# erererq/gym-lorenz

Hardware: NVIDIA B200
Metric: env_steps_per_sec (higher is better)
Workload: dtype f64

## Files before the change

gym_lorenz_b200/csrc/chaos_b200.cu:

```cuda
#include <math.h>
#include <pthread.h>
#include <sched.h>
#include <stdarg.h>
#include <time.h>
#include <stdio.h>
#include <stdlib.h>
#include <string.h>

#include "kernels_common.cuh"
#include "host_copy.h"

cudaError_t cl_launch_derivatives(int kind, const void* state, const float* action, void* out,
                                  int64_t n, cudaStream_t st);

using cl::KParams;

struct CopyHelper;

namespace {

const cl_layout kLayouts[CL_ENV_KIND_COUNT] = {
     {8, 4, 0, 6, 3, 0, -500.0, 500.0, -HUGE_VAL, HUGE_VAL, 0, 0},
     {8, 10, 0, 6, 3, 0, -500.0, 500.0, -HUGE_VAL, HUGE_VAL, 0, 0},
     {8, 9, 0, 8, 3, 0, -2.0, 2.0, -HUGE_VAL, HUGE_VAL, 0, 0},
// ... 306 lines not shown
  if (r == CL_OK) ctx->step_index += 1;
  return r;
}

extern "C" int cl_step(cl_ctx* ctx, void* stream, const cl_buffers* buf, const cl_io* io) {
  if (!ctx) return fail(nullptr, CL_EINVAL, "null ctx");
  if (!io || !io->action) return fail(ctx, CL_EINVAL, "cl_step: io.action is required");
  KParams p;
  int r = fill_params(ctx, buf, io, p);
  if (r) return r;
  p.reward_f32 = 0;
  CU(cudaSetDevice(ctx->cfg.device));
  r = launch(ctx, p, cl::MODE_STEP, (cudaStream_t)stream);
  if (r == CL_OK) ctx->step_index += 1;
  return r;
}

typedef CUresult (*encode_tiled_fn)(CUtensorMap*, CUtensorMapDataType, cuuint32_t, void*, const cuuint64_t*,
                                    const cuuint64_t*, const cuuint32_t*, const cuuint32_t*, CUtensorMapInterleave,
                                    CUtensorMapSwizzle, CUtensorMapL2promotion, CUtensorMapFloatOOBfill);
static bool action_tensor_map(CUtensorMap* out, const float* base, uint64_t n_x, uint64_t n_ch, uint64_t T,
                              uint64_t row_stride, uint64_t t_stride, uint32_t chunk) {
  static encode_tiled_fn fn = nullptr;
  static bool tried = false;
  if (!tried) {
    tried = true;
    void* f = nullptr;
    cudaDriverEntryPointQueryResult q;
    if (cudaGetDriverEntryPoint("cuTensorMapEncodeTiled", &f, cudaEnableDefault, &q) == cudaSuccess &&
        q == cudaDriverEntryPointSuccess)
      fn = (encode_tiled_fn)f;
  }
  if (!fn || chunk < 1 || chunk > 256 || n_ch > 256 || T < chunk) return false;
  const cuuint64_t dims[3] = {n_x, n_ch, T};
  const cuuint64_t strides[2] = {row_stride * sizeof(float), t_stride * sizeof(float)};
  const cuuint32_t box[3] = {32, (cuuint32_t)n_ch, chunk};
  const cuuint32_t estr[3] = {1, 1, 1};
  return fn(out, CU_TENSOR_MAP_DATA_TYPE_FLOAT32, 3, (void*)base, dims, strides, box, estr, CU_TENSOR_MAP_INTERLEAVE_NONE,
            CU_TENSOR_MAP_SWIZZLE_NONE, CU_TENSOR_MAP_L2_PROMOTION_NONE, CU_TENSOR_MAP_FLOAT_OOB_FILL_NONE) == CUDA_SUCCESS;
}

static bool want_dynamic(const cl_ctx* ctx, int T, int chunk) {
  const char* ov = getenv("CHAOS_B200_DYN");
  if (ov && ov[0] == '0') return false;
  const int64_t W = (ctx->cfg.num_envs + 31) / 32, nsched = (int64_t)ctx->sm_count * 4;
  if (T < 2 * chunk) return false;
  if (ov && ov[0] == '1') return true;
  if (W <= nsched) return false;
  if (W * (int64_t)((T + chunk - 1) / chunk) >= (int64_t)1 << 31) return false;
  const double eff = (double)W / (double)(((W + nsched - 1) / nsched) * nsched);
  return eff < 0.95;
}

extern "C" int cl_rollout(cl_ctx* ctx, void* stream, const cl_buffers* buf, const cl_io* io,
                          const cl_rollout_desc* d) {
  if (!ctx) return fail(nullptr, CL_EINVAL, "null ctx");
  if (!io || !d || d->T < 1) return fail(ctx, CL_EINVAL, "cl_rollout: io/desc required, T >= 1");
  if (io->noise) return fail(ctx, CL_EINVAL, "cl_rollout: noise override is single-step only");
  KParams p;
  int r = fill_params(ctx, buf, io, p);
  if (r) return r;
  p.T = d->T; p.act_ts = d->act_ts; p.obs_ts = d->obs_ts; p.rew_ts = d->rew_ts; p.done_ts = d->done_ts;
  p.synth_amp = (float)d->synth_amp;
  cudaStream_t st = (cudaStream_t)stream;
  CU(cudaSetDevice(ctx->cfg.device));
  int chunk = CL_DYN_CHUNK_DEFAULT;
  if (const char* ov = getenv("CHAOS_B200_DYN_CHUNK")) { const int c = atoi(ov); if (c >= 1 && c <= 16) chunk = c; }
  int mode = cl::MODE_ROLLOUT;
  alignas(64) CUtensorMap tmap;
  if (want_dynamic(ctx, d->T, chunk)) {
    const int64_t W = (ctx->cfg.num_envs + 31) / 32;
    if (!ctx->dyn_bps) {
      int occ = 0;
      cudaError_t e = is_parity(ctx->cfg.kind) ? cl_dyn_occupancy_parity(ctx->cfg.kind, chunk, &occ)
                                               : cl_dyn_occupancy_northstar(ctx->cfg.kind, chunk, &occ);
      if (e != cudaSuccess) return fail(ctx, CL_ECUDA, "dyn occupancy query: %s", cudaGetErrorString(e));
      int bps = (int)(W / ((int64_t)ctx->sm_count * 4));
      bps = bps < 1 ? 1 : (bps > 4 ? 4 : bps);
      if (const char* ov = getenv("CHAOS_B200_DYN_BPS")) { const int b = atoi(ov); if (b >= 1 && b <= 16) bps = b; }
      ctx->dyn_bps = occ < bps ? occ : bps;
    }
    if (ctx->dyn_bps >= 1) {
      CU(cudaMemsetAsync(ctx->d_dyn, 0, sizeof(uint32_t) * (size_t)(W + 1), st));
      p.dyn_counter = ctx->d_dyn;
      p.dyn_progress = ctx->d_dyn + 1;
      p.dyn_chunk = chunk;
      p.dyn_nchunks = (d->T + chunk - 1) / chunk;
      p.dyn_nwarps = (int32_t)W;
      const int64_t workers = (int64_t)ctx->sm_count * ctx->dyn_bps;
      const int64_t tasks = W * (int64_t)((d->T + chunk - 1) / chunk);
      p.dyn_grid = (int32_t)(workers * 4 < tasks ? workers : (tasks + 3) / 4);
      p.dyn_tma = (io->action != nullptr && io->act_es == 1 && (io->act_cs % 4) == 0 && (d->act_ts % 4) == 0 &&
                   ((uintptr_t)io->action % 16) == 0 && io->act_cs >= W * 32) ? 1 : 0;
      {
        const char* ov = getenv("CHAOS_B200_SM");
        if (!(ov && ov[0] == '0') && p.dyn_tma) {
          const int grid = (int)(W < ctx->sm_count ? W : ctx->sm_count);
          const int qn = (int)(W / grid), cmax = (int)((W + grid - 1) / grid);
          int workers = qn >= 4 ? 4 * (qn / 4) : qn;
          workers = workers > 16 ? 16 : workers;
          if (workers == 16 && qn < 20) workers = 12;
          if (const char* w = getenv("CHAOS_B200_SM_WORKERS")) { const int k = atoi(w); if (k >= 1 && k <= 16) workers = k < qn ? k : qn; }
          int sc = 16;
          const size_t per_warp = (size_t)ctx->lay.n_state * 32u * (size_t)ctx->lay.real_bytes + 32u * 12u + 28u;
          while (sc > 1 && (size_t)cmax * (2u * (size_t)sc * (size_t)ctx->lay.act_dim * 128u + per_warp) + 256u > 200u * 1024u) sc /= 2;
          if (const char* w = getenv("CHAOS_B200_SM_CHUNK")) { const int k = atoi(w); if (k >= 1 && k <= 16) sc = k; }
          if (sc > d->T) sc = d->T;
          if (cmax <= 64) {
            p.sm_grid = grid; p.sm_workers = workers; p.sm_chunk = sc;
            p.sm_gdiv = 1;
            if (const char* w = getenv("CHAOS_B200_SM_GDIV")) { const int k = atoi(w); if (k >= 1 && k <= 16) p.sm_gdiv = k; }
            p.host_tmap = &tmap;
            p.sm_tmap_ok = action_tensor_map(&tmap, io->action, (uint64_t)W * 32, (uint64_t)ctx->lay.act_dim,
                                             (uint64_t)d->T, (uint64_t)io->act_cs, (uint64_t)d->act_ts, (uint32_t)sc) ? 1 : 0;
            const char* tm = getenv("CHAOS_B200_SM_TMAP");
            if (tm && tm[0] == '0') p.sm_tmap_ok = 0;
          }
        }
      }
      mode = cl::MODE_ROLLOUT_DYN;
      ctx->dyn_launches += 1;
    }
  }
  r = launch(ctx, p, mode, st);
  if (r == CL_OK) ctx->step_index += (uint64_t)d->T;
  return r;
}

static int check_policy_kind(cl_ctx* ctx, const char* fn, int kind) {
  if (kind == CL_ENV_HR_SYNC || kind == CL_ENV_PMSM_SYNC) return CL_OK;
  return fail(ctx, CL_EINVAL, "%s: env kind %d is not supported (hr_sync and pmsm_sync only)", fn, kind);
}

static int policy_prelude(cl_ctx* ctx, const char* fn, const char* objs, bool objs_ok, const cl_io* io,
                          const cl_rollout_desc* d, const cl_policy* pol, bool need_last) {
  if (!ctx) return fail(nullptr, CL_EINVAL, "null ctx");
  const int r = check_policy_kind(ctx, fn, ctx->cfg.kind);
  if (r) return r;
  if (ctx->cfg.flags & CL_F_OBS_F64) return fail(ctx, CL_EINVAL, "%s: float32 observations only", fn);
  if (!io || !d || !pol || !objs_ok || d->T < 1) return fail(ctx, CL_EINVAL, "%s: %s required, T >= 1", fn, objs);
  if (io->action || io->noise) return fail(ctx, CL_EINVAL, "%s: io.action and io.noise must be NULL", fn);
  if (!pol->params || !pol->obs0 || (need_last && !pol->obs_last))
    return fail(ctx, CL_EINVAL, need_last ? "%s: params, obs0 and obs_last are required"
                                          : "%s: params and obs0 are required", fn);
  return CL_OK;
}

static int policy_params(cl_ctx* ctx, const cl_buffers* buf, const cl_io* io, const cl_rollout_desc* d,
                         KParams& p) {
  const int r = fill_params(ctx, buf, io, p);
  if (r) return r;
  p.T = d->T; p.obs_ts = d->obs_ts; p.rew_ts = d->rew_ts; p.done_ts = d->done_ts;
  CU(cudaSetDevice(ctx->cfg.device));
  return CL_OK;
}

static bool collect_complete(const cl_collect* col) {
  return col->starts && col->obs && col->actions && col->rewards && col->values && col->log_probs &&
         col->episode_starts && col->last_values;
}

static int policy_done(cl_ctx* ctx, cudaStream_t st, cudaError_t e, const char* what, int T) {
  if (e != cudaSuccess) return fail(ctx, CL_ECUDA, "%s launch failed: %s", what, cudaGetErrorString(e));
  ctx->launches += 1;
// ... 497 lines not shown
```

gym_lorenz_b200/csrc/kernels_common.cuh:

```cuda
#pragma once
#include <cuda.h>
#include <cuda_runtime.h>
#include <stdint.h>
#include <string.h>

#include "../../include/chaos_b200.h"
#include "philox.cuh"

namespace cl {

struct KParams {
  int64_t n, n_pad, env_id_base;
  int64_t i_begin;
  uint32_t k0, k1;
  uint64_t step_index;
  uint64_t* step_ptr;
  int32_t max_steps, substeps, flags, reward_f32;
  double dt, alpha, act_limit, act_gain, param_jitter;
  void* state;
  int32_t* aux_int;
  int32_t* ep_len;
  double* ep_return;
  double* stats;
  const float* action;
  int64_t act_es, act_cs;
  const double* noise;
  void* obs;
  int64_t obs_es, obs_cs;
  void* reward;
  uint8_t* done;
  void* term_obs;
  double* last_ep_ret;
  int32_t* last_ep_len;
  const uint8_t* mask;
  uint8_t* warp_done;
  int32_t host_rows;
  const uint32_t* act_ready;
  uint32_t act_gen;
  int32_t act_slice_envs;
  int32_t act_lane_slices;
  const uint32_t* act_host_words;
  int32_t act_lanes, act_nslices;
  uint32_t* host_err;
  int32_t T;
  int64_t act_ts, obs_ts, rew_ts, done_ts;
  float synth_amp;
  const float* bc1;
  const float* bc2;
  int32_t bc1_n, bc2_n;
  double h, hh, h3, h6;
  float hf, hhf, h3f, h6f;
  double nom[3];
  float nomf[3];
  double nom_br;
  float nom_brf;
  float act_limit_f, act_gain_f;
  uint32_t* dyn_counter;
  uint32_t* dyn_progress;
  int32_t dyn_chunk, dyn_nchunks, dyn_nwarps, dyn_tma, dyn_grid;
  int32_t sm_grid, sm_workers, sm_chunk, sm_gdiv;
  int32_t sm_tmap_ok;
  const CUtensorMap* host_tmap;
  int32_t rows_fast;
  int32_t no_plain;
  int32_t* host_plain_out;
};

enum LaunchMode { MODE_STEP = 0, MODE_ROLLOUT = 1, MODE_RESET = 2, MODE_INIT = 3, MODE_ROLLOUT_DYN = 4 };


__device__ __forceinline__ float clipf(float a, float lo, float hi) {
  return a < lo ? lo : (a > hi ? hi : a);
}
__device__ __forceinline__ double clipd(double a, double lo, double hi) {
  return a < lo ? lo : (a > hi ? hi : a);
}

__device__ __forceinline__ double pow_pos(double x, double a) {
  if (a == 0.5) return sqrt(x);
  if (a == 1.0 / 3) return cbrt(x);
  if (!(a > 0.0) || !(a < 64.0)) return pow(x, a);
  if (x == 0.0) return 0.0;
  return exp(a * log(x));
}

__device__ __forceinline__ double mul_keep(double a, double b) { return __dmul_rn(a, b); }
__device__ __forceinline__ float mul_keep(float a, float b) { return a * b; }
__device__ __forceinline__ double mul_rn(double a, double b) { return __dmul_rn(a, b); }
__device__ __forceinline__ float mul_rn(float a, float b) { return __fmul_rn(a, b); }

__device__ __forceinline__ Stream make_stream(const KParams& p, int64_t i, uint64_t step) {
  const uint64_t gid = (uint64_t)(p.env_id_base + i);
  Stream s;
  s.id_lo = (uint32_t)gid;
  s.id_hi = (uint32_t)(gid >> 32);
  s.step = (uint32_t)step;
  s.k0 = p.k0;
  s.k1 = p.k1 ^ (uint32_t)((step >> 32) & 0x00FFFFFFu);
  return s;
}

__device__ __forceinline__ uint64_t step_base(const KParams& p) {
  return p.step_ptr != nullptr ? *((volatile const uint64_t*)p.step_ptr) : p.step_index;
}
__global__ void k_advance_step(uint64_t* step, uint64_t count);
__global__ void k_relay(const uint32_t* host_words, uint32_t* dev_words, uint32_t gen, uint32_t lanes, uint32_t spl,
                        uint32_t nslices, uint32_t* host_err);

template <int N>
__device__ __forceinline__ void draw_uniform(const Stream& rng, uint32_t tag, double lo, double hi,
                                             double* out) {
#pragma unroll
  for (int b = 0; b < (N + 1) / 2; ++b) {
    const u32x4 r = rng.draw(tag + (uint32_t)b);
    out[2 * b] = uniform53(r.x, r.y, lo, hi);
    if (2 * b + 1 < N) out[2 * b + 1] = uniform53(r.z, r.w, lo, hi);
  }
}
// ... 560 lines not shown
      phase ^= 1u;
    }
    const float* ab = abuf;
    unsigned bad_acc = 0u;
    bool fin = E::finite(s);
    PlainPending<E> pend;
    pend.begin(p, i, t0);
    auto intervals = [&](auto spec_tag) {
      constexpr int SPEC = decltype(spec_tag)::value;
      for (int tl = 0; tl < len; ++tl) {
        const int t = t0 + tl;
        const uint64_t step = step0 + (uint64_t)t;
        float a[E::ACT];
        if (!PLAIN && p.action == nullptr) {
          synth_action<E>(p, make_stream(p, i, step), a);
        } else if (tma) {
#pragma unroll
          for (int cc = 0; cc < E::ACT; ++cc) a[cc] = ab[(tl * E::ACT + cc) * 32 + lane];
        } else {
#pragma unroll
          for (int cc = 0; cc < E::ACT; ++cc)
            a[cc] = live ? p.action[(int64_t)t * p.act_ts + i * p.act_es + cc * p.act_cs] : 0.0f;
        }
        env_interval<E, true, PLAIN, SPEC, true>(s, ep_len, ep_ret, p, i, live, lane, t, step, a, want_noise, obs64, autoreset, bad_acc, sm_rows, fin, &pend);
      }
    };
    if constexpr (PLAIN) {
      if (E::spec(s, p) == 1) intervals(SpecTag<1>{});
      else intervals(SpecTag<0>{});
    } else {
      intervals(SpecTag<0>{});
    }
    if (bad_acc && lane == 0) atomicAdd(&p.stats[CL_STAT_NONFINITE], (double)bad_acc);
    bad_acc = 0u;
    if (live) {
      E::store(s, p, i);
      p.ep_len[i] = ep_len;
      p.ep_return[i] = ep_ret;
    }
    __syncwarp();
    if (lane == 0) st_release_u32(p.dyn_progress + e, c + 1u);
    if constexpr (PLAIN) {
      if (CL_PLAIN_DEFER) plain_emit<E, true>(p, i, live, pend);
    }
    q = grab();
  }
}



template <class E>
struct SmLayout {
  typedef typename E::real real;
  size_t act, state, ep_ret, ep_len, mbar, prog, total;
  __host__ __device__ SmLayout(int cnt, int chunk) {
    size_t o = 0;
    act = o;    o += (size_t)cnt * 2 * chunk * E::ACT * 32 * sizeof(float);
    state = o;  o += (size_t)cnt * E::NSTATE * 32 * sizeof(real);
    ep_ret = o; o += (size_t)cnt * 32 * sizeof(double);
    ep_len = o; o += (size_t)cnt * 32 * sizeof(int32_t);
    mbar = o;   o += (size_t)cnt * 3 * sizeof(uint64_t);
    prog = o;   o += ((size_t)cnt + 1) * sizeof(uint32_t);
    total = (o + 127) & ~(size_t)127;
  }
};

__device__ __forceinline__ void tma_load_3d(void* dst, const void* tmap, int x, int y, int z, uint64_t* bar) {
  asm volatile(
      "cp.async.bulk.tensor.3d.shared::cluster.global.tile.mbarrier::complete_tx::bytes [%0], [%1, {%2, %3, %4}], [%5];"
      ::"r"(smem_u32(dst)), "l"(tmap), "r"(x), "r"(y), "r"(z), "r"(smem_u32(bar))
      : "memory");
}

#ifndef CL_SM_THREADS
#define CL_SM_THREADS 576
#endif
#ifndef CL_SM_MINB
#define CL_SM_MINB 0
#endif
template <class E>
__global__ void __launch_bounds__(CL_SM_THREADS, CL_SM_MINB) k_rollout_sm(const KParams p,
                                                                         const __grid_constant__ CUtensorMap tmap) {
  typedef typename E::real real;
  extern __shared__ __align__(128) unsigned char sm_raw[];
  const unsigned lane = threadIdx.x & 31u;
  const int wib = threadIdx.x >> 5, nres = blockDim.x >> 5;
  const int W = p.dyn_nwarps, G = (int)gridDim.x, b = (int)blockIdx.x;
  const int qn = W / G, rn = W % G;
  const int e0 = b * qn + (b < rn ? b : rn);
  const int cnt = qn + (b < rn ? 1 : 0);
  const int cmax = qn + (rn ? 1 : 0);
  const int ng = cnt - nres;
  const int Tc = p.sm_chunk, Tg = max(1, Tc / max(1, p.sm_gdiv));
  const int nchunks = 1 + (p.T - 1 + Tc - 1) / Tc;
  const int nchunks_g = 1 + (p.T - 1 + Tg - 1) / Tg;
  auto chunk_t0 = [&](int f, int c, int tc) { return c == 0 ? 0 : min(p.T, f + (c - 1) * tc); };
  auto chunk_len = [&](int f, int c, int tc) { return min(c == 0 ? f : tc, p.T - chunk_t0(f, c, tc)); };
  const SmLayout<E> L(cmax, Tc);
  float* const act = (float*)(sm_raw + L.act);
  real* const st = (real*)(sm_raw + L.state);
  double* const s_ret = (double*)(sm_raw + L.ep_ret);
  int32_t* const s_len = (int32_t*)(sm_raw + L.ep_len);
  uint64_t* const mbar = (uint64_t*)(sm_raw + L.mbar);
  volatile uint32_t* const prog = (volatile uint32_t*)(sm_raw + L.prog);
  uint32_t* const counter = (uint32_t*)(sm_raw + L.prog) + cmax;
  const int per_buf = Tc * E::ACT * 32;

  for (int k = threadIdx.x; k < cnt * 3; k += blockDim.x) mbar_init(&mbar[k], 1);
  for (int k = threadIdx.x; k <= cmax; k += blockDim.x) ((uint32_t*)(sm_raw + L.prog))[k] = 0u;
  for (int k = threadIdx.x; k < cnt * 32; k += blockDim.x) {
    const int le = k >> 5, ln = k & 31;
    const int64_t i = (int64_t)(e0 + le) * 32 + ln;
#pragma unroll
    for (int c = 0; c < E::NSTATE; ++c) st[(le * E::NSTATE + c) * 32 + ln] = ldp<real>(p, c, i);
    s_ret[k] = __ldcg(p.ep_return + i);
    s_len[k] = __ldcg(p.ep_len + i);
  }
  asm volatile("fence.mbarrier_init.release.cluster;" ::: "memory");
  __syncthreads();

  auto stage = [&](int le, int f, int c, int tc) {
    const int t0 = chunk_t0(f, c, tc);
    uint64_t* bar = &mbar[le * 3 + (c & 1)];
    float* dst = act + (size_t)(le * 2 + (c & 1)) * per_buf;
    if (p.sm_tmap_ok) {
      if (lane == 0) {
        mbar_expect_tx(bar, (uint32_t)(per_buf * sizeof(float)));
        tma_load_3d(dst, &tmap, (e0 + le) * 32, 0, t0, bar);
      }
    } else {
      const int len = chunk_len(f, c, tc);
      if (lane == 0) mbar_expect_tx(bar, (uint32_t)(len * E::ACT * 128));
      __syncwarp();
      for (int k = (int)lane; k < len * E::ACT; k += 32) {
        const int tl = k / E::ACT, cc = k % E::ACT;
        const float* src = p.action + (int64_t)(t0 + tl) * p.act_ts + (int64_t)cc * p.act_cs + (int64_t)(e0 + le) * 32;
        bulk_g2s(dst + (tl * E::ACT + cc) * 32, src, 128u, bar);
      }
    }
  };
  auto wait_actions = [&](int le, int c) {
    uint64_t* bar = &mbar[le * 3 + (c & 1)];
    const uint32_t parity = (uint32_t)(c >> 1) & 1u;
    uint32_t spins = 0;
    while (!mbar_try_wait(bar, parity)) spin_guard(spins);
  };
  for (int le = wib; le < cnt; le += nres) { const int tc = le < nres ? Tc : Tg; stage(le, 1 + le * tc / cnt, 0, tc); }

  const uint64_t step0 = step_base(p);
  unsigned bad_acc = 0u;

  auto run_chunk = [&](typename E::S& s, int32_t& ep_len, double& ep_ret, bool& fin, PlainPending<E>& pend,
                       const int le, const int c, const int t0, const int len, const int64_t i, const bool live) {
    const float* ab = act + (size_t)(le * 2 + (c & 1)) * per_buf;
    auto intervals = [&](auto spec_tag) {
      constexpr int SPEC = decltype(spec_tag)::value;
      for (int tl = 0; tl < len; ++tl) {
        const int t = t0 + tl;
        const uint64_t step = step0 + (uint64_t)t;
        float a[E::ACT];
#pragma unroll
        for (int cc = 0; cc < E::ACT; ++cc) a[cc] = ab[(tl * E::ACT + cc) * 32 + lane];
        env_interval<E, true, true, SPEC, true>(s, ep_len, ep_ret, p, i, live, lane, t, step, a, false, false, true,
                                                bad_acc, nullptr, fin, &pend);
      }
    };
    if (E::spec(s, p) == 1) intervals(SpecTag<1>{});
    else intervals(SpecTag<0>{});
  };

  const uint32_t g_total = (uint32_t)ng * (uint32_t)nchunks_g;
  const int g_credit = ng * (Tc / Tg);
  typename E::S s = {};
  int32_t ep_len = 0;
  double ep_ret = 0.0;
  bool fin = true;
  PlainPending<E> pend;
  pend.valid = 0u;
  int in_regs = -1;
  int c_own = 0;
  int credit = (wib * g_credit) % nres;
  bool guests_left = ng > 0, want_guest = false;
  for (;;) {
    int le, c;
    bool guest;
    if (want_guest) {
      uint32_t q = 0;
      if (lane == 0) q = atomicAdd(counter, 1u);
      q = __shfl_sync(0xffffffffu, q, 0);
      if (q >= g_total) { guests_left = false; want_guest = false; continue; }
      guest = true; le = nres + (int)(q % (uint32_t)ng); c = (int)(q / (uint32_t)ng);
    } else if (c_own < nchunks) {
      guest = false; le = wib; c = c_own;
    } else if (guests_left) {
      want_guest = true;
      continue;
    } else {
      break;
    }
    const int tc = guest ? Tg : Tc, nch = guest ? nchunks_g : nchunks;
    const int f = 1 + le * tc / cnt;
    const int t0 = chunk_t0(f, c, tc), len = chunk_len(f, c, tc);
    const int64_t i = (int64_t)(e0 + le) * 32 + lane;
    const bool live = i < p.n;
    if (guest && c > 0) {
      uint32_t spins = 0;
      if (lane == 0) {
        while (prog[le] != (uint32_t)c) { __nanosleep(32); spin_guard(spins); }
      }
      __syncwarp();
      uint64_t* hb = &mbar[le * 3 + 2];
      const uint32_t parity = (uint32_t)(c - 1) & 1u;
      while (!mbar_try_wait(hb, parity)) spin_guard(spins);
    }
    if (c + 1 < nch) stage(le, f, c + 1, tc);
    if (in_regs != le) {
      E::load_sm(s, st + (size_t)le * E::NSTATE * 32, lane);
      ep_len = s_len[le * 32 + lane];
      ep_ret = s_ret[le * 32 + lane];
      E::prepare(s, p, live);
      fin = E::finite(s);
      pend.begin(p, i, t0);
      in_regs = le;
    }
    wait_actions(le, c);
    run_chunk(s, ep_len, ep_ret, fin, pend, le, c, t0, len, i, live);
    bool park;
    if (guest) {
      park = true;
      want_guest = false;
    } else {
      c_own += 1;
      credit += g_credit;
      want_guest = guests_left && credit >= nres && c_own < nchunks;
      if (want_guest) credit -= nres;
      park = want_guest || c_own == nchunks;
    }
    if (park) {
      E::store_sm(s, st + (size_t)le * E::NSTATE * 32, lane);
      s_len[le * 32 + lane] = ep_len;
      s_ret[le * 32 + lane] = ep_ret;
      if (guest) {
        __syncwarp();
        if (lane == 0) {
          prog[le] = (uint32_t)c + 1u;
          mbar_arrive(&mbar[le * 3 + 2]);
        }
      }
      if (CL_PLAIN_DEFER) plain_emit<E, true>(p, i, live, pend);
      pend.valid = 0u;
      in_regs = -1;
    }
  }
  if (bad_acc && lane == 0) atomicAdd(&p.stats[CL_STAT_NONFINITE], (double)bad_acc);

  __syncthreads();
  for (int k = threadIdx.x; k < cnt * 32; k += blockDim.x) {
    const int le = k >> 5, ln = k & 31;
    const int64_t i = (int64_t)(e0 + le) * 32 + ln;
    if (i < p.n) {
#pragma unroll
      for (int c = 0; c < E::NSTATE; ++c) stp<real>(p, c, i, st[(le * E::NSTATE + c) * 32 + ln]);
      p.ep_return[i] = s_ret[k];
      p.ep_len[i] = s_len[k];
    }
  }
}

template <class E>
__global__ void __launch_bounds__(256) k_reset(const KParams p) {
  typedef typename E::real real;
  const int64_t i = (int64_t)blockIdx.x * blockDim.x + threadIdx.x;
  const uint64_t step0 = step_base(p);
  if (i < p.n && (p.mask == nullptr || p.mask[i] != 0)) {
    typename E::S s = {};
    E::load(s, p, i);
    const Stream rng = make_stream(p, i, step0);
    real obs[E::OBS];
    E::reset(s, p, rng, obs);
    E::store(s, p, i);
    p.ep_len[i] = 0;
    p.ep_return[i] = 0.0;
    if (p.obs) store_obs<real>(p.obs, 0, p.obs_es, p.obs_cs, i, obs, E::OBS, (p.flags & CL_F_OBS_F64) != 0);
  }
}

template <class E>
__global__ void __launch_bounds__(256) k_init(const KParams p) {
  const int64_t i = (int64_t)blockIdx.x * blockDim.x + threadIdx.x;
  if (i >= p.n) return;
  typename E::S s = {};
  const Stream rng = make_stream(p, i, 0);
  E::init_persistent(s, p, rng);
  E::store(s, p, i);
  p.ep_len[i] = 0;
  p.ep_return[i] = 0.0;
}

template <class E>
inline bool rows_fast_ok(const KParams& p, bool rollout) {
  return p.obs != nullptr && !(p.flags & CL_F_OBS_F64) && p.obs_cs == 1 && p.obs_es == E::OBS &&
         ((uintptr_t)p.obs % 16) == 0 && (!rollout || (p.obs_ts % 4) == 0) &&
         ((uintptr_t)p.term_obs % 16) == 0;
}

template <class E>
inline bool plain_rollout_ok(const KParams& p, int mode) {
  return PlainRollout<E>::value && !p.no_plain && E::NOISE == 0 && p.action != nullptr && p.obs != nullptr && p.obs_es == 1 &&
         p.obs_cs == p.n_pad && p.obs_ts == (int64_t)E::OBS * p.n_pad && p.rew_ts == p.n_pad && p.done_ts == p.n_pad &&
         !(p.flags & CL_F_OBS_F64) && !p.rows_fast && p.reward != nullptr && !p.reward_f32 && p.done != nullptr &&
         p.term_obs == nullptr &&
         (p.flags & CL_F_AUTORESET) && (mode != MODE_ROLLOUT_DYN || p.dyn_tma);
}

template <class E>
cudaError_t launch_env(const KParams& p_in, int mode, cudaStream_t st, int block) {
  KParams p = p_in;
  const bool roll = (mode == MODE_ROLLOUT || mode == MODE_ROLLOUT_DYN);
  p.rows_fast = (mode == MODE_STEP || roll) && rows_fast_ok<E>(p, roll) ? 1 : 0;
  constexpr bool HAS_PLAIN = PlainRollout<E>::value != 0;
  const bool plain = roll && plain_rollout_ok<E>(p, mode);
  if (p.host_plain_out) *p.host_plain_out = plain ? 1 : 0;
  p.host_plain_out = nullptr;
  const size_t row_smem = p.rows_fast ? (size_t)(block / 32) * 32 * E::OBS * sizeof(float) : 0;
  const unsigned grid = (unsigned)((p.n - p.i_begin + block - 1) / block);
  const unsigned step_grid = grid + ((mode == MODE_STEP && p.act_host_words != nullptr) ? 1u : 0u);
  switch (mode) {
    case MODE_STEP: k_step<E, false><<<step_grid, block, row_smem, st>>>(p); break;
    case MODE_ROLLOUT:
      if (plain) k_step<E, true, HAS_PLAIN><<<grid, block, row_smem, st>>>(p);
      else k_step<E, true><<<grid, block, row_smem, st>>>(p);
      break;
    case MODE_RESET: k_reset<E><<<grid, block, 0, st>>>(p); break;
    case MODE_INIT: k_init<E><<<grid, block, 0, st>>>(p); break;
    case MODE_ROLLOUT_DYN: {
      if constexpr (HAS_PLAIN) {
        if (plain && p.sm_grid > 0) {
          const int cmax = (p.dyn_nwarps + p.sm_grid - 1) / p.sm_grid;
          size_t smem = SmLayout<E>(cmax, p.sm_chunk).total;
          if (smem < 120 * 1024) smem = 120 * 1024;
          if (smem <= 200 * 1024) {
            static bool attr_set = false;
            if (!attr_set) {
              cudaError_t e = cudaFuncSetAttribute(k_rollout_sm<E>, cudaFuncAttributeMaxDynamicSharedMemorySize, 200 * 1024);
              if (e != cudaSuccess) return e;
              attr_set = true;
            }
            if (p_in.host_plain_out) *p_in.host_plain_out |= 2;
            alignas(64) CUtensorMap tm;
            if (p.sm_tmap_ok && p.host_tmap) tm = *p.host_tmap;
            else { memset(&tm, 0, sizeof(tm)); p.sm_tmap_ok = 0; }
            p.host_tmap = nullptr;
            k_rollout_sm<E><<<(unsigned)p.sm_grid, (unsigned)p.sm_workers * 32, smem, st>>>(p, tm);
            break;
          }
        }
      }
      const size_t smem = (size_t)4 * p.dyn_chunk * E::ACT * 32 * sizeof(float) + 4 * sizeof(uint64_t);
      if (plain) k_rollout_dyn<E, HAS_PLAIN><<<(unsigned)p.dyn_grid, 128, smem, st>>>(p);
      else k_rollout_dyn<E><<<(unsigned)p.dyn_grid, 128, smem, st>>>(p);
      break;
    }
    default: return cudaErrorInvalidValue;
  }
  return cudaGetLastError();
}

template <class E>
cudaError_t dyn_occupancy(int chunk, int* blocks_per_sm) {
  const size_t smem = (size_t)4 * chunk * E::ACT * 32 * sizeof(float) + 4 * sizeof(uint64_t);
  cudaError_t e = cudaFuncSetAttribute(k_rollout_dyn<E>, cudaFuncAttributePreferredSharedMemoryCarveout, 50);
  if (e != cudaSuccess) return e;
  int occ = 0, occ_plain = 1 << 30;
  e = cudaOccupancyMaxActiveBlocksPerMultiprocessor(&occ, k_rollout_dyn<E>, 128, smem);
  if (e != cudaSuccess) return e;
  if (PlainRollout<E>::value) {
    e = cudaFuncSetAttribute(k_rollout_dyn<E, PlainRollout<E>::value != 0>, cudaFuncAttributePreferredSharedMemoryCarveout, 50);
    if (e != cudaSuccess) return e;
    e = cudaOccupancyMaxActiveBlocksPerMultiprocessor(&occ_plain, k_rollout_dyn<E, PlainRollout<E>::value != 0>, 128, smem);
    if (e != cudaSuccess) return e;
  }
  *blocks_per_sm = occ < occ_plain ? occ : occ_plain;
  return cudaSuccess;
}

}

cudaError_t cl_launch_parity(int kind, const cl::KParams& p, int mode, cudaStream_t st, int block);
cudaError_t cl_launch_northstar(int kind, const cl::KParams& p, int mode, cudaStream_t st, int block);
cudaError_t cl_occupancy_parity(int kind, int block, int* blocks_per_sm);
cudaError_t cl_occupancy_northstar(int kind, int block, int* blocks_per_sm);
cudaError_t cl_dyn_occupancy_parity(int kind, int chunk, int* blocks_per_sm);
cudaError_t cl_dyn_occupancy_northstar(int kind, int chunk, int* blocks_per_sm);
cudaError_t cl_launch_policy(int kind, const cl::KParams& p, const cl_policy& q, float act_lo, float act_hi,
                             cudaStream_t st, int sms);
cudaError_t cl_launch_policy_collect(int kind, const cl::KParams& p, const cl_policy& q, const cl_collect& col,
                                     float act_lo, float act_hi, cudaStream_t st, int sms);
cudaError_t cl_launch_policy_collect_norm(int kind, const cl::KParams& p, const cl_policy& q, const cl_collect& col,
                                          const cl_vecnorm_update& vn, float act_lo, float act_hi, cudaStream_t st,
                                          int sms);
int64_t cl_policy_collect_norm_bytes(int obs_dim, int64_t n);
cudaError_t cl_fma_peak_launch(int dtype_bytes, int grid, int block, int iters, void* sink, cudaStream_t st);
```

gym_lorenz_b200/csrc/tu_northstar.cu:

```cuda
#include "envs_northstar.cuh"

using namespace cl;

#define CL_NS_KINDS(X)                              \
  X(CL_ENV_LORENZ_RK4, EnvLorenzRK4<double>)        \
  X(CL_ENV_LORENZ_RK4_F32, EnvLorenzRK4<float>)     \
  X(CL_ENV_PMSM_RK4, EnvPMSMRK4)

cudaError_t cl_launch_northstar(int kind, const KParams& p, int mode, cudaStream_t st, int block) {
  switch (kind) {
#define X(K, E) case K: return launch_env<E>(p, mode, st, block);
    CL_NS_KINDS(X)
#undef X
    default: return cudaErrorInvalidValue;
  }
}

cudaError_t cl_occupancy_northstar(int kind, int block, int* out) {
  switch (kind) {
#define X(K, E) case K: return cudaOccupancyMaxActiveBlocksPerMultiprocessor(out, k_step<E, true>, block, 0);
    CL_NS_KINDS(X)
#undef X
    default: return cudaErrorInvalidValue;
  }
}

cudaError_t cl_dyn_occupancy_northstar(int kind, int chunk, int* out) {
  switch (kind) {
#define X(K, E) case K: return dyn_occupancy<E>(chunk, out);
    CL_NS_KINDS(X)
#undef X
    default: return cudaErrorInvalidValue;
  }
}

template <typename R>
__global__ void __launch_bounds__(256) k_fma_peak(int iters, R* sink) {
  R a[8];
  const R m = R(1.0) - R(1e-7), c = R(1e-9);
#pragma unroll
  for (int j = 0; j < 8; ++j) a[j] = R(threadIdx.x + j) * R(1e-3);
  for (int it = 0; it < iters; ++it) {
#pragma unroll
    for (int r = 0; r < 16; ++r) {
#pragma unroll
      for (int j = 0; j < 8; ++j) a[j] = fma(a[j], m, c);
    }
  }
  R s = R(0);
#pragma unroll
  for (int j = 0; j < 8; ++j) s += a[j];
  if (s == R(-1.2345)) sink[0] = s;
}

cudaError_t cl_fma_peak_launch(int dtype_bytes, int grid, int block, int iters, void* sink, cudaStream_t st) {
  if (dtype_bytes == 8) k_fma_peak<double><<<grid, block, 0, st>>>(iters, (double*)sink);
  else k_fma_peak<float><<<grid, block, 0, st>>>(iters, (float*)sink);
  return cudaGetLastError();
}
```

Before: 21.70 billion.

## Replace guest-chunk work stealing with static split of env-step span across warps

Drops the dynamic guest/credit work-stealing scheme in the shared-memory rollout kernel, where extra warps' chunks were claimed through an atomic counter and progress flags. Each resident warp now gets a contiguous slice of the flattened (env × timestep) span, with weights that can differ by warp rank. Any env split between two warps hands off through an mbarrier. This removes the atomic counter, progress polling and guest chunk subdivision, but the static balance may leave warps idle if work is uneven. Optional globaltimer probe instrumentation is also added behind a compile flag.

Result: faster. 22.05 billion (median of 6 runs) (+1.6%).

```diff
diff --git a/gym_lorenz_b200/csrc/chaos_b200.cu b/gym_lorenz_b200/csrc/chaos_b200.cu
--- a/gym_lorenz_b200/csrc/chaos_b200.cu
+++ b/gym_lorenz_b200/csrc/chaos_b200.cu
@@ -432,14 +432,12 @@
           if (workers == 16 && qn < 20) workers = 12;
           if (const char* w = getenv("CHAOS_B200_SM_WORKERS")) { const int k = atoi(w); if (k >= 1 && k <= 16) workers = k < qn ? k : qn; }
           int sc = 16;
-          const size_t per_warp = (size_t)ctx->lay.n_state * 32u * (size_t)ctx->lay.real_bytes + 32u * 12u + 28u;
+          const size_t per_warp = (size_t)ctx->lay.n_state * 32u * (size_t)ctx->lay.real_bytes + 32u * 12u + 24u;
           while (sc > 1 && (size_t)cmax * (2u * (size_t)sc * (size_t)ctx->lay.act_dim * 128u + per_warp) + 256u > 200u * 1024u) sc /= 2;
           if (const char* w = getenv("CHAOS_B200_SM_CHUNK")) { const int k = atoi(w); if (k >= 1 && k <= 16) sc = k; }
           if (sc > d->T) sc = d->T;
           if (cmax <= 64) {
             p.sm_grid = grid; p.sm_workers = workers; p.sm_chunk = sc;
-            p.sm_gdiv = 1;
-            if (const char* w = getenv("CHAOS_B200_SM_GDIV")) { const int k = atoi(w); if (k >= 1 && k <= 16) p.sm_gdiv = k; }
             p.host_tmap = &tmap;
             p.sm_tmap_ok = action_tensor_map(&tmap, io->action, (uint64_t)W * 32, (uint64_t)ctx->lay.act_dim,
                                              (uint64_t)d->T, (uint64_t)io->act_cs, (uint64_t)d->act_ts, (uint32_t)sc) ? 1 : 0;
diff --git a/gym_lorenz_b200/csrc/kernels_common.cuh b/gym_lorenz_b200/csrc/kernels_common.cuh
--- a/gym_lorenz_b200/csrc/kernels_common.cuh
+++ b/gym_lorenz_b200/csrc/kernels_common.cuh
@@ -58,7 +58,7 @@
   uint32_t* dyn_counter;
   uint32_t* dyn_progress;
   int32_t dyn_chunk, dyn_nchunks, dyn_nwarps, dyn_tma, dyn_grid;
-  int32_t sm_grid, sm_workers, sm_chunk, sm_gdiv;
+  int32_t sm_grid, sm_workers, sm_chunk;
   int32_t sm_tmap_ok;
   const CUtensorMap* host_tmap;
   int32_t rows_fast;
@@ -730,7 +730,7 @@
 template <class E>
 struct SmLayout {
   typedef typename E::real real;
-  size_t act, state, ep_ret, ep_len, mbar, prog, total;
+  size_t act, state, ep_ret, ep_len, mbar, total;
   __host__ __device__ SmLayout(int cnt, int chunk) {
     size_t o = 0;
     act = o;    o += (size_t)cnt * 2 * chunk * E::ACT * 32 * sizeof(float);
@@ -738,7 +738,6 @@
     ep_ret = o; o += (size_t)cnt * 32 * sizeof(double);
     ep_len = o; o += (size_t)cnt * 32 * sizeof(int32_t);
     mbar = o;   o += (size_t)cnt * 3 * sizeof(uint64_t);
-    prog = o;   o += ((size_t)cnt + 1) * sizeof(uint32_t);
     total = (o + 127) & ~(size_t)127;
   }
 };
@@ -753,9 +752,26 @@
 #ifndef CL_SM_THREADS
 #define CL_SM_THREADS 576
 #endif
+#ifndef CL_SM_RANK_W
+#define CL_SM_RANK_W 1
+#endif
 #ifndef CL_SM_MINB
 #define CL_SM_MINB 0
 #endif
+#ifdef CL_SM_PROBE
+#define CL_SM_PROBE_STRIDE 18
+__device__ unsigned long long cl_sm_probe_buf[256 * CL_SM_PROBE_STRIDE];
+__device__ __forceinline__ unsigned long long globaltimer_ns() {
+  unsigned long long t;
+  asm volatile("mov.u64 %0, %globaltimer;" : "=l"(t));
+  return t;
+}
+#define CL_SM_PROBE_AT(slot) \
+  if (lane == 0 && blockIdx.x < 256) cl_sm_probe_buf[blockIdx.x * CL_SM_PROBE_STRIDE + (slot)] = globaltimer_ns()
+#else
+#define CL_SM_PROBE_AT(slot)
+#endif
+
 template <class E>
 __global__ void __launch_bounds__(CL_SM_THREADS, CL_SM_MINB) k_rollout_sm(const KParams p,
                                                                          const __grid_constant__ CUtensorMap tmap) {
@@ -768,24 +784,19 @@
   const int e0 = b * qn + (b < rn ? b : rn);
   const int cnt = qn + (b < rn ? 1 : 0);
   const int cmax = qn + (rn ? 1 : 0);
-  const int ng = cnt - nres;
-  const int Tc = p.sm_chunk, Tg = max(1, Tc / max(1, p.sm_gdiv));
-  const int nchunks = 1 + (p.T - 1 + Tc - 1) / Tc;
-  const int nchunks_g = 1 + (p.T - 1 + Tg - 1) / Tg;
-  auto chunk_t0 = [&](int f, int c, int tc) { return c == 0 ? 0 : min(p.T, f + (c - 1) * tc); };
-  auto chunk_len = [&](int f, int c, int tc) { return min(c == 0 ? f : tc, p.T - chunk_t0(f, c, tc)); };
+  const int Tc = p.sm_chunk;
+  auto chunk_t0 = [&](int f, int c) { return c == 0 ? 0 : min(p.T, f + (c - 1) * Tc); };
+  auto chunk_len = [&](int f, int c) { return min(c == 0 ? f : Tc, p.T - chunk_t0(f, c)); };
+  if (threadIdx.x == 0) { CL_SM_PROBE_AT(0); }
   const SmLayout<E> L(cmax, Tc);
   float* const act = (float*)(sm_raw + L.act);
   real* const st = (real*)(sm_raw + L.state);
   double* const s_ret = (double*)(sm_raw + L.ep_ret);
   int32_t* const s_len = (int32_t*)(sm_raw + L.ep_len);
   uint64_t* const mbar = (uint64_t*)(sm_raw + L.mbar);
-  volatile uint32_t* const prog = (volatile uint32_t*)(sm_raw + L.prog);
-  uint32_t* const counter = (uint32_t*)(sm_raw + L.prog) + cmax;
   const int per_buf = Tc * E::ACT * 32;
 
   for (int k = threadIdx.x; k < cnt * 3; k += blockDim.x) mbar_init(&mbar[k], 1);
-  for (int k = threadIdx.x; k <= cmax; k += blockDim.x) ((uint32_t*)(sm_raw + L.prog))[k] = 0u;
   for (int k = threadIdx.x; k < cnt * 32; k += blockDim.x) {
     const int le = k >> 5, ln = k & 31;
     const int64_t i = (int64_t)(e0 + le) * 32 + ln;
@@ -797,8 +808,8 @@
   asm volatile("fence.mbarrier_init.release.cluster;" ::: "memory");
   __syncthreads();
 
-  auto stage = [&](int le, int f, int c, int tc) {
-    const int t0 = chunk_t0(f, c, tc);
+  auto stage = [&](int le, int f, int c) {
+    const int t0 = chunk_t0(f, c);
     uint64_t* bar = &mbar[le * 3 + (c & 1)];
     float* dst = act + (size_t)(le * 2 + (c & 1)) * per_buf;
     if (p.sm_tmap_ok) {
@@ -807,7 +818,7 @@
         tma_load_3d(dst, &tmap, (e0 + le) * 32, 0, t0, bar);
       }
     } else {
-      const int len = chunk_len(f, c, tc);
+      const int len = chunk_len(f, c);
       if (lane == 0) mbar_expect_tx(bar, (uint32_t)(len * E::ACT * 128));
       __syncwarp();
       for (int k = (int)lane; k < len * E::ACT; k += 32) {
@@ -823,14 +834,13 @@
     uint32_t spins = 0;
     while (!mbar_try_wait(bar, parity)) spin_guard(spins);
   };
-  for (int le = wib; le < cnt; le += nres) { const int tc = le < nres ? Tc : Tg; stage(le, 1 + le * tc / cnt, 0, tc); }
+  for (int le = wib; le < cnt; le += nres) stage(le, 1 + le * Tc / cnt, 0);
 
   const uint64_t step0 = step_base(p);
   unsigned bad_acc = 0u;
 
   auto run_chunk = [&](typename E::S& s, int32_t& ep_len, double& ep_ret, bool& fin, PlainPending<E>& pend,
-                       const int le, const int c, const int t0, const int len, const int64_t i, const bool live) {
-    const float* ab = act + (size_t)(le * 2 + (c & 1)) * per_buf;
+                       const float* ab, const int t0, const int len, const int64_t i, const bool live) {
     auto intervals = [&](auto spec_tag) {
       constexpr int SPEC = decltype(spec_tag)::value;
       for (int tl = 0; tl < len; ++tl) {
@@ -847,89 +857,74 @@
     else intervals(SpecTag<0>{});
   };
 
-  const uint32_t g_total = (uint32_t)ng * (uint32_t)nchunks_g;
-  const int g_credit = ng * (Tc / Tg);
+  const int64_t span = (int64_t)cnt * p.T;
+  const int nr = (nres + 3) >> 2;
+  auto prefix = [&](int w, int step) -> int64_t {
+    int64_t s = 0;
+    for (int v = 0; v < w; ++v) s += 128 + step * (2 * (v >> 2) - (nr - 1));
+    return s;
+  };
+  int step = CL_SM_RANK_W;
+  if (span * (128 - step * (nr - 1)) < (int64_t)(p.T + 1) * prefix(nres, step)) step = 0;
+  const int64_t wtot = prefix(nres, step);
+  int64_t x = span * prefix(wib, step) / wtot;
+  const int64_t x_end = span * prefix(wib + 1, step) / wtot;
   typename E::S s = {};
   int32_t ep_len = 0;
   double ep_ret = 0.0;
   bool fin = true;
   PlainPending<E> pend;
   pend.valid = 0u;
-  int in_regs = -1;
-  int c_own = 0;
-  int credit = (wib * g_credit) % nres;
-  bool guests_left = ng > 0, want_guest = false;
+  int le = -1, f = 1, t = 0, t_end = 0;
+  bool early = false;
+  int64_t i = 0;
+  bool live = false;
   for (;;) {
-    int le, c;
-    bool guest;
-    if (want_guest) {
-      uint32_t q = 0;
-      if (lane == 0) q = atomicAdd(counter, 1u);
-      q = __shfl_sync(0xffffffffu, q, 0);
-      if (q >= g_total) { guests_left = false; want_guest = false; continue; }
-      guest = true; le = nres + (int)(q % (uint32_t)ng); c = (int)(q / (uint32_t)ng);
-    } else if (c_own < nchunks) {
-      guest = false; le = wib; c = c_own;
-    } else if (guests_left) {
-      want_guest = true;
-      continue;
-    } else {
-      break;
-    }
-    const int tc = guest ? Tg : Tc, nch = guest ? nchunks_g : nchunks;
-    const int f = 1 + le * tc / cnt;
-    const int t0 = chunk_t0(f, c, tc), len = chunk_len(f, c, tc);
-    const int64_t i = (int64_t)(e0 + le) * 32 + lane;
-    const bool live = i < p.n;
-    if (guest && c > 0) {
-      uint32_t spins = 0;
-      if (lane == 0) {
-        while (prog[le] != (uint32_t)c) { __nanosleep(32); spin_guard(spins); }
-      }
-      __syncwarp();
-      uint64_t* hb = &mbar[le * 3 + 2];
-      const uint32_t parity = (uint32_t)(c - 1) & 1u;
-      while (!mbar_try_wait(hb, parity)) spin_guard(spins);
-    }
-    if (c + 1 < nch) stage(le, f, c + 1, tc);
-    if (in_regs != le) {
+    if (t == t_end) {
+      if (le >= 0) {
+        E::store_sm(s, st + (size_t)le * E::NSTATE * 32, lane);
+        s_len[le * 32 + lane] = ep_len;
+        s_ret[le * 32 + lane] = ep_ret;
+        if (early) {
+          __syncwarp();
+          if (lane == 0) mbar_arrive(&mbar[le * 3 + 2]);
+        }
+        if (CL_PLAIN_DEFER) plain_emit<E, true>(p, i, live, pend);
+        pend.valid = 0u;
+      }
+      if (x >= x_end) break;
+      le = (int)(x / p.T);
+      const int64_t lo = x, hi = min(x_end, (int64_t)(le + 1) * p.T);
+      const int len = (int)(hi - lo);
+      early = lo > (int64_t)le * p.T;
+      const bool late = hi < (int64_t)(le + 1) * p.T;
+      t = late ? p.T - len : 0;
+      t_end = t + len;
+      x = hi;
+      f = 1 + le * Tc / cnt;
+      i = (int64_t)(e0 + le) * 32 + lane;
+      live = i < p.n;
+      if (late) {
+        uint32_t spins = 0;
+        while (!mbar_try_wait(&mbar[le * 3 + 2], 0u)) spin_guard(spins);
+      }
       E::load_sm(s, st + (size_t)le * E::NSTATE * 32, lane);
       ep_len = s_len[le * 32 + lane];
       ep_ret = s_ret[le * 32 + lane];
       E::prepare(s, p, live);
       fin = E::finite(s);
-      pend.begin(p, i, t0);
-      in_regs = le;
-    }
+      pend.begin(p, i, t);
+    }
+    const int c = t < f ? 0 : 1 + (t - f) / Tc;
+    const int c_t0 = chunk_t0(f, c), c_end = c_t0 + chunk_len(f, c);
+    if (t == c_t0 && c_end < p.T) stage(le, f, c + 1);
     wait_actions(le, c);
-    run_chunk(s, ep_len, ep_ret, fin, pend, le, c, t0, len, i, live);
-    bool park;
-    if (guest) {
-      park = true;
-      want_guest = false;
-    } else {
-      c_own += 1;
-      credit += g_credit;
-      want_guest = guests_left && credit >= nres && c_own < nchunks;
-      if (want_guest) credit -= nres;
-      park = want_guest || c_own == nchunks;
-    }
-    if (park) {
-      E::store_sm(s, st + (size_t)le * E::NSTATE * 32, lane);
-      s_len[le * 32 + lane] = ep_len;
-      s_ret[le * 32 + lane] = ep_ret;
-      if (guest) {
-        __syncwarp();
-        if (lane == 0) {
-          prog[le] = (uint32_t)c + 1u;
-          mbar_arrive(&mbar[le * 3 + 2]);
-        }
-      }
-      if (CL_PLAIN_DEFER) plain_emit<E, true>(p, i, live, pend);
-      pend.valid = 0u;
-      in_regs = -1;
-    }
-  }
+    const int len = min(c_end, t_end) - t;
+    run_chunk(s, ep_len, ep_ret, fin, pend, act + (size_t)(le * 2 + (c & 1)) * per_buf + (size_t)(t - c_t0) * E::ACT * 32,
+              t, len, i, live);
+    t += len;
+  }
+  CL_SM_PROBE_AT(2 + wib);
   if (bad_acc && lane == 0) atomicAdd(&p.stats[CL_STAT_NONFINITE], (double)bad_acc);
 
   __syncthreads();
@@ -943,6 +938,10 @@
       p.ep_len[i] = s_len[k];
     }
   }
+#ifdef CL_SM_PROBE
+  __syncthreads();
+  if (threadIdx.x == 0) { CL_SM_PROBE_AT(1); }
+#endif
 }
 
 template <class E>
diff --git a/gym_lorenz_b200/csrc/tu_northstar.cu b/gym_lorenz_b200/csrc/tu_northstar.cu
--- a/gym_lorenz_b200/csrc/tu_northstar.cu
+++ b/gym_lorenz_b200/csrc/tu_northstar.cu
@@ -58,3 +58,10 @@
   else k_fma_peak<float><<<grid, block, 0, st>>>(iters, (float*)sink);
   return cudaGetLastError();
 }
+
+#ifdef CL_SM_PROBE
+extern "C" int cl_sm_probe_read(unsigned long long* host, int n) {
+  if (n < 0 || n > 256 * CL_SM_PROBE_STRIDE) return (int)cudaErrorInvalidValue;
+  return (int)cudaMemcpyFromSymbol(host, cl::cl_sm_probe_buf, (size_t)n * sizeof(unsigned long long));
+}
+#endif
```

## Use programmatic dependent launch and early TMA staging in shared-memory rollout kernel

Applied to the files above, without the earlier changes.

Launches the shared-memory rollout kernel with programmatic stream serialization so its prologue can overlap the previous kernel's tail. In f64 builds, lane 0 of each warp initializes its own mbarriers and issues the first action TMA loads right after griddepcontrol.wait, before the state loads into shared memory. The dyn counter memset is moved so it runs only for the fallback dyn kernel, which removes one memset launch on the shared-memory path. This relies on griddepcontrol ordering being correct and on the shared-memory kernel never using the dyn counter.

Result: faster. 21.69 billion before, 21.95 billion after, median of 6 (+1.2%).

```diff
diff --git a/gym_lorenz_b200/csrc/chaos_b200.cu b/gym_lorenz_b200/csrc/chaos_b200.cu
--- a/gym_lorenz_b200/csrc/chaos_b200.cu
+++ b/gym_lorenz_b200/csrc/chaos_b200.cu
@@ -411,7 +411,6 @@
       ctx->dyn_bps = occ < bps ? occ : bps;
     }
     if (ctx->dyn_bps >= 1) {
-      CU(cudaMemsetAsync(ctx->d_dyn, 0, sizeof(uint32_t) * (size_t)(W + 1), st));
       p.dyn_counter = ctx->d_dyn;
       p.dyn_progress = ctx->d_dyn + 1;
       p.dyn_chunk = chunk;
diff --git a/gym_lorenz_b200/csrc/kernels_common.cuh b/gym_lorenz_b200/csrc/kernels_common.cuh
--- a/gym_lorenz_b200/csrc/kernels_common.cuh
+++ b/gym_lorenz_b200/csrc/kernels_common.cuh
@@ -784,19 +784,6 @@
   uint32_t* const counter = (uint32_t*)(sm_raw + L.prog) + cmax;
   const int per_buf = Tc * E::ACT * 32;
 
-  for (int k = threadIdx.x; k < cnt * 3; k += blockDim.x) mbar_init(&mbar[k], 1);
-  for (int k = threadIdx.x; k <= cmax; k += blockDim.x) ((uint32_t*)(sm_raw + L.prog))[k] = 0u;
-  for (int k = threadIdx.x; k < cnt * 32; k += blockDim.x) {
-    const int le = k >> 5, ln = k & 31;
-    const int64_t i = (int64_t)(e0 + le) * 32 + ln;
-#pragma unroll
-    for (int c = 0; c < E::NSTATE; ++c) st[(le * E::NSTATE + c) * 32 + ln] = ldp<real>(p, c, i);
-    s_ret[k] = __ldcg(p.ep_return + i);
-    s_len[k] = __ldcg(p.ep_len + i);
-  }
-  asm volatile("fence.mbarrier_init.release.cluster;" ::: "memory");
-  __syncthreads();
-
   auto stage = [&](int le, int f, int c, int tc) {
     const int t0 = chunk_t0(f, c, tc);
     uint64_t* bar = &mbar[le * 3 + (c & 1)];
@@ -823,7 +810,45 @@
     uint32_t spins = 0;
     while (!mbar_try_wait(bar, parity)) spin_guard(spins);
   };
-  for (int le = wib; le < cnt; le += nres) { const int tc = le < nres ? Tc : Tg; stage(le, 1 + le * tc / cnt, 0, tc); }
+
+  constexpr bool EARLY_COPIES = sizeof(real) == 8;
+  asm volatile("griddepcontrol.launch_dependents;" ::: "memory");
+  if constexpr (EARLY_COPIES) {
+    if (lane == 0) {
+      for (int le = wib; le < cnt; le += nres) {
+        mbar_init(&mbar[le * 3 + 0], 1); mbar_init(&mbar[le * 3 + 1], 1); mbar_init(&mbar[le * 3 + 2], 1);
+      }
+      asm volatile("fence.mbarrier_init.release.cluster;" ::: "memory");
+    }
+    __syncwarp();
+    asm volatile("griddepcontrol.wait;" ::: "memory");
+    for (int le = wib; le < cnt; le += nres) { const int tc = le < nres ? Tc : Tg; stage(le, 1 + le * tc / cnt, 0, tc); }
+    for (int k = threadIdx.x; k <= cmax; k += blockDim.x) ((uint32_t*)(sm_raw + L.prog))[k] = 0u;
+    for (int k = threadIdx.x; k < cnt * 32; k += blockDim.x) {
+      const int le = k >> 5, ln = k & 31;
+      const int64_t i = (int64_t)(e0 + le) * 32 + ln;
+#pragma unroll
+      for (int c = 0; c < E::NSTATE; ++c) st[(le * E::NSTATE + c) * 32 + ln] = ldp<real>(p, c, i);
+      s_ret[k] = __ldcg(p.ep_return + i);
+      s_len[k] = __ldcg(p.ep_len + i);
+    }
+    __syncthreads();
+  } else {
+    asm volatile("griddepcontrol.wait;" ::: "memory");
+    for (int k = threadIdx.x; k < cnt * 3; k += blockDim.x) mbar_init(&mbar[k], 1);
+    for (int k = threadIdx.x; k <= cmax; k += blockDim.x) ((uint32_t*)(sm_raw + L.prog))[k] = 0u;
+    for (int k = threadIdx.x; k < cnt * 32; k += blockDim.x) {
+      const int le = k >> 5, ln = k & 31;
+      const int64_t i = (int64_t)(e0 + le) * 32 + ln;
+#pragma unroll
+      for (int c = 0; c < E::NSTATE; ++c) st[(le * E::NSTATE + c) * 32 + ln] = ldp<real>(p, c, i);
+      s_ret[k] = __ldcg(p.ep_return + i);
+      s_len[k] = __ldcg(p.ep_len + i);
+    }
+    asm volatile("fence.mbarrier_init.release.cluster;" ::: "memory");
+    __syncthreads();
+    for (int le = wib; le < cnt; le += nres) { const int tc = le < nres ? Tc : Tg; stage(le, 1 + le * tc / cnt, 0, tc); }
+  }
 
   const uint64_t step0 = step_base(p);
   unsigned bad_acc = 0u;
@@ -1029,10 +1054,23 @@
             if (p.sm_tmap_ok && p.host_tmap) tm = *p.host_tmap;
             else { memset(&tm, 0, sizeof(tm)); p.sm_tmap_ok = 0; }
             p.host_tmap = nullptr;
-            k_rollout_sm<E><<<(unsigned)p.sm_grid, (unsigned)p.sm_workers * 32, smem, st>>>(p, tm);
-            break;
+            cudaLaunchConfig_t cfg = {};
+            cfg.gridDim = dim3((unsigned)p.sm_grid);
+            cfg.blockDim = dim3((unsigned)p.sm_workers * 32);
+            cfg.dynamicSmemBytes = smem;
+            cfg.stream = st;
+            cudaLaunchAttribute attr[1];
+            attr[0].id = cudaLaunchAttributeProgrammaticStreamSerialization;
+            attr[0].val.programmaticStreamSerializationAllowed = 1;
+            cfg.attrs = attr;
+            cfg.numAttrs = 1;
+            return cudaLaunchKernelEx(&cfg, k_rollout_sm<E>, p, tm);
           }
         }
+      }
+      {
+        const cudaError_t e = cudaMemsetAsync(p.dyn_counter, 0, sizeof(uint32_t) * ((size_t)p.dyn_nwarps + 1), st);
+        if (e != cudaSuccess) return e;
       }
       const size_t smem = (size_t)4 * p.dyn_chunk * E::ACT * 32 * sizeof(float) + 4 * sizeof(uint64_t);
       if (plain) k_rollout_dyn<E, HAS_PLAIN><<<(unsigned)p.dyn_grid, 128, smem, st>>>(p);
```

## Launch SM rollout with programmatic dependent launch and skip its counter memset

Applied to the files above, without the earlier changes.

Moves the dynamic-counter memset so it runs only on the k_rollout_dyn fallback path, which removes an extra memset from the shared-memory rollout path. The shared-memory kernel is now launched with programmatic stream serialization, and it calls griddepcontrol.wait and launch_dependents, so its prologue can overlap the tail of the previous kernel. It also adds an optional, compile-time-disabled timeline instrumentation buffer using globaltimer and clock64. The risk is that correctness now depends on the SM kernel initialising its own counters in shared memory, which it appears to do.

Result: no change. 21.64 billion before, 21.82 billion after, median of 6 (+0.9%).

```diff
diff --git a/gym_lorenz_b200/csrc/chaos_b200.cu b/gym_lorenz_b200/csrc/chaos_b200.cu
--- a/gym_lorenz_b200/csrc/chaos_b200.cu
+++ b/gym_lorenz_b200/csrc/chaos_b200.cu
@@ -382,6 +382,16 @@
   return eff < 0.95;
 }
 
+#if CL_SM_TIMELINE
+static uint64_t* g_tl = nullptr;
+static int32_t g_tl_cap = 0;
+extern "C" int cl_sm_timeline(void* buf, int32_t cap) {
+  g_tl = (uint64_t*)buf;
+  g_tl_cap = cap;
+  return CL_OK;
+}
+#endif
+
 extern "C" int cl_rollout(cl_ctx* ctx, void* stream, const cl_buffers* buf, const cl_io* io,
                           const cl_rollout_desc* d) {
   if (!ctx) return fail(nullptr, CL_EINVAL, "null ctx");
@@ -390,6 +400,10 @@
   KParams p;
   int r = fill_params(ctx, buf, io, p);
   if (r) return r;
+#if CL_SM_TIMELINE
+  p.tl = g_tl;
+  p.tl_cap = g_tl_cap;
+#endif
   p.T = d->T; p.act_ts = d->act_ts; p.obs_ts = d->obs_ts; p.rew_ts = d->rew_ts; p.done_ts = d->done_ts;
   p.synth_amp = (float)d->synth_amp;
   cudaStream_t st = (cudaStream_t)stream;
@@ -411,7 +425,6 @@
       ctx->dyn_bps = occ < bps ? occ : bps;
     }
     if (ctx->dyn_bps >= 1) {
-      CU(cudaMemsetAsync(ctx->d_dyn, 0, sizeof(uint32_t) * (size_t)(W + 1), st));
       p.dyn_counter = ctx->d_dyn;
       p.dyn_progress = ctx->d_dyn + 1;
       p.dyn_chunk = chunk;
diff --git a/gym_lorenz_b200/csrc/kernels_common.cuh b/gym_lorenz_b200/csrc/kernels_common.cuh
--- a/gym_lorenz_b200/csrc/kernels_common.cuh
+++ b/gym_lorenz_b200/csrc/kernels_common.cuh
@@ -6,6 +6,10 @@
 
 #include "../../include/chaos_b200.h"
 #include "philox.cuh"
+
+#ifndef CL_SM_TIMELINE
+#define CL_SM_TIMELINE 0
+#endif
 
 namespace cl {
 
@@ -64,6 +68,10 @@
   int32_t rows_fast;
   int32_t no_plain;
   int32_t* host_plain_out;
+#if CL_SM_TIMELINE
+  uint64_t* tl;
+  int32_t tl_cap;
+#endif
 };
 
 enum LaunchMode { MODE_STEP = 0, MODE_ROLLOUT = 1, MODE_RESET = 2, MODE_INIT = 3, MODE_ROLLOUT_DYN = 4 };
@@ -752,6 +760,19 @@
 
 #ifndef CL_SM_THREADS
 #define CL_SM_THREADS 576
+#endif
+#if CL_SM_TIMELINE
+constexpr int TL_BLK = 16, TL_WHDR = 4, TL_REC = 6;
+__device__ __forceinline__ uint64_t tl_gtime() {
+  uint64_t t;
+  asm volatile("mov.u64 %0, %%globaltimer;" : "=l"(t));
+  return t;
+}
+__device__ __forceinline__ uint64_t tl_smid() {
+  uint32_t s;
+  asm volatile("mov.u32 %0, %%smid;" : "=r"(s));
+  return s;
+}
 #endif
 #ifndef CL_SM_MINB
 #define CL_SM_MINB 0
@@ -784,6 +805,20 @@
   uint32_t* const counter = (uint32_t*)(sm_raw + L.prog) + cmax;
   const int per_buf = Tc * E::ACT * 32;
 
+  asm volatile("griddepcontrol.wait;" ::: "memory");
+#if CL_SM_TIMELINE
+  uint64_t* const tlb = p.tl ? p.tl + (size_t)b * TL_BLK : nullptr;
+  auto tl_worker = [&]() {
+    return p.tl + (size_t)G * TL_BLK + ((size_t)b * nres + wib) * (TL_WHDR + (size_t)p.tl_cap * TL_REC);
+  };
+  if (p.tl && lane == 0) tl_worker()[0] = 0;
+  if (tlb && threadIdx.x == 0) {
+    tlb[0] = tl_smid() | (uint64_t)cnt << 32 | (uint64_t)nres << 48;
+    tlb[1] = tl_gtime();
+    tlb[6] = clock64();
+  }
+#endif
+
   for (int k = threadIdx.x; k < cnt * 3; k += blockDim.x) mbar_init(&mbar[k], 1);
   for (int k = threadIdx.x; k <= cmax; k += blockDim.x) ((uint32_t*)(sm_raw + L.prog))[k] = 0u;
   for (int k = threadIdx.x; k < cnt * 32; k += blockDim.x) {
@@ -796,6 +831,10 @@
   }
   asm volatile("fence.mbarrier_init.release.cluster;" ::: "memory");
   __syncthreads();
+#if CL_SM_TIMELINE
+  if (tlb && threadIdx.x == 0) { tlb[2] = tl_gtime(); tlb[7] = clock64(); }
+#endif
+  asm volatile("griddepcontrol.launch_dependents;" ::: "memory");
 
   auto stage = [&](int le, int f, int c, int tc) {
     const int t0 = chunk_t0(f, c, tc);
@@ -881,6 +920,12 @@
     const int t0 = chunk_t0(f, c, tc), len = chunk_len(f, c, tc);
     const int64_t i = (int64_t)(e0 + le) * 32 + lane;
     const bool live = i < p.n;
+#if CL_SM_TIMELINE
+    if (p.tl && lane == 0 && tl_worker()[0] < (uint64_t)p.tl_cap) {
+      uint64_t* r = tl_worker() + TL_WHDR + (size_t)tl_worker()[0] * TL_REC;
+      r[1] = tl_gtime(); r[3] = clock64();
+    }
+#endif
     if (guest && c > 0) {
       uint32_t spins = 0;
       if (lane == 0) {
@@ -929,7 +974,19 @@
       pend.valid = 0u;
       in_regs = -1;
     }
-  }
+#if CL_SM_TIMELINE
+    if (p.tl && lane == 0 && tl_worker()[0] < (uint64_t)p.tl_cap) {
+      uint64_t* const w = tl_worker();
+      uint64_t* r = w + TL_WHDR + (size_t)w[0] * TL_REC;
+      r[0] = (uint64_t)le | (uint64_t)c << 8 | (uint64_t)guest << 16 | (uint64_t)len << 24 | (uint64_t)t0 << 40;
+      r[2] = tl_gtime(); r[4] = clock64(); r[5] = 0;
+      w[0] += 1;
+    }
+#endif
+  }
+#if CL_SM_TIMELINE
+  if (p.tl && lane == 0) { uint64_t* const w = tl_worker(); w[1] = tl_gtime(); w[2] = clock64(); w[3] = 0; }
+#endif
   if (bad_acc && lane == 0) atomicAdd(&p.stats[CL_STAT_NONFINITE], (double)bad_acc);
 
   __syncthreads();
@@ -943,6 +1000,18 @@
       p.ep_len[i] = s_len[k];
     }
   }
+#if CL_SM_TIMELINE
+  if (tlb && threadIdx.x == 0) {
+    uint64_t g_lo = ~0ull, g_hi = 0, c_lo = ~0ull, c_hi = 0;
+    for (int w = 0; w < nres; ++w) {
+      const uint64_t* h = p.tl + (size_t)G * TL_BLK + ((size_t)b * nres + w) * (TL_WHDR + (size_t)p.tl_cap * TL_REC);
+      g_lo = min(g_lo, h[1]); g_hi = max(g_hi, h[1]); c_lo = min(c_lo, h[2]); c_hi = max(c_hi, h[2]);
+    }
+    tlb[3] = g_lo; tlb[4] = g_hi; tlb[8] = c_lo; tlb[9] = c_hi;
+  }
+  __syncthreads();
+  if (tlb && threadIdx.x == 0) { tlb[5] = tl_gtime(); tlb[10] = clock64(); }
+#endif
 }
 
 template <class E>
@@ -1029,10 +1098,25 @@
             if (p.sm_tmap_ok && p.host_tmap) tm = *p.host_tmap;
             else { memset(&tm, 0, sizeof(tm)); p.sm_tmap_ok = 0; }
             p.host_tmap = nullptr;
-            k_rollout_sm<E><<<(unsigned)p.sm_grid, (unsigned)p.sm_workers * 32, smem, st>>>(p, tm);
+            cudaLaunchConfig_t cfg = {};
+            cfg.gridDim = dim3((unsigned)p.sm_grid);
+            cfg.blockDim = dim3((unsigned)p.sm_workers * 32);
+            cfg.dynamicSmemBytes = smem;
+            cfg.stream = st;
+            cudaLaunchAttribute attr[1];
+            attr[0].id = cudaLaunchAttributeProgrammaticStreamSerialization;
+            attr[0].val.programmaticStreamSerializationAllowed = 1;
+            cfg.attrs = attr;
+            cfg.numAttrs = 1;
+            cudaError_t e = cudaLaunchKernelEx(&cfg, k_rollout_sm<E>, p, tm);
+            if (e != cudaSuccess) return e;
             break;
           }
         }
+      }
+      {
+        const cudaError_t e = cudaMemsetAsync(p.dyn_counter, 0, sizeof(uint32_t) * ((size_t)p.dyn_nwarps + 1), st);
+        if (e != cudaSuccess) return e;
       }
       const size_t smem = (size_t)4 * p.dyn_chunk * E::ACT * 32 * sizeof(float) + 4 * sizeof(uint64_t);
       if (plain) k_rollout_dyn<E, HAS_PLAIN><<<(unsigned)p.dyn_grid, 128, smem, st>>>(p);
```
